# xmindflow/TransCeption

Measured on AMD Instinct MI355X. Metric: images/sec fwd+bwd at 224x224 B=16 per GPU, higher is better.
Workload: dtype bf16; 1 GPU; TransCeption (MSTransception) 224x224 B=16/GPU fwd+bwd+SGD, synthetic Synapse npz slices via the device loader, name-seeded random-init weights; global_batch=16, image_size=224, parallelism=dp1, headline_mode=loader, headline_degraded=False, launch_mode=hipGraph replay

## Files before the change

### transception_amd/_header.py

```python
from __future__ import annotations

import ctypes as C
import operator
import os
import re
from typing import NamedTuple

HEADER = os.path.join(os.path.dirname(os.path.dirname(os.path.abspath(__file__))), "include", "transception_hip.h")


class SideHeader(NamedTuple):
    attr: str
    file: str
    version: str
    entry: str
    what: str

    @property
    def path(self) -> str:
        return os.path.join(os.path.dirname(HEADER), self.file)


SIDE_HEADERS = (SideHeader("POST", "transception_post.h", "TC_POST_ABI_VERSION", "tc_post_abi_version", "post-processing"),
                SideHeader("EMA", "transception_ema.h", "TC_EMA_ABI_VERSION", "tc_ema_abi_version", "weight-averaging"),
                SideHeader("TTA", "transception_tta.h", "TC_TTA_ABI_VERSION", "tc_tta_abi_version", "test-time augmentation"),
                SideHeader("RESAMPLE", "transception_resample.h", "TC_RESAMPLE_ABI_VERSION", "tc_resample_abi_version", "score resampling"),
                SideHeader("BRIDGE", "transception_bridge.h", "TC_BRIDGE_ABI_VERSION", "tc_bridge_abi_version", "bridge LayerNorm"),
                SideHeader("LOSS", "transception_loss.h", "TC_LOSS_ABI_VERSION", "tc_loss_abi_version", "focal / Tversky loss"))

SCALARS = {"int": C.c_int, "long long": C.c_longlong, "float": C.c_float, "double": C.c_double,
           "unsigned": C.c_uint, "unsigned int": C.c_uint}
POINTEES = set(SCALARS) | {"void", "unsigned char"}


class HeaderError(ValueError):
    pass


class Function(NamedTuple):
    restype: type
    argtypes: list
    query: bool


class Header(NamedTuple):
    functions: dict
    structs: dict
    constants: dict


_TOKEN = re.compile(r"\s*(\d+|<<|[()|+-])")
_LEVELS = ({"|": operator.or_}, {"<<": operator.lshift}, {"+": operator.add, "-": operator.sub})


def evaluate(expr: str) -> int:
    toks, pos, expr = [], 0, expr.strip()
    while pos < len(expr):
        m = _TOKEN.match(expr, pos)
        if not m:
            raise HeaderError(f"constant expression {expr!r}: cannot read {expr[pos:]!r}")
# ... 122 lines not shown
```

### transception_amd/_lib.py

```python
from __future__ import annotations

import ctypes as C
import os

from . import _header

HERE = os.path.dirname(os.path.abspath(__file__))
LIB_PATH = os.environ.get("TC_LIB_PATH") or os.path.join(HERE, "libtransception_hip.so")

ABI = _header.load()
SIGNATURES = {name: f.argtypes for name, f in ABI.functions.items()}
K, S = ABI.constants, ABI.structs
SIDE = {s.attr: _header.load(s.path) for s in _header.SIDE_HEADERS}
POST, EMA, TTA, RESAMPLE, BRIDGE, LOSS = SIDE["POST"], SIDE["EMA"], SIDE["TTA"], SIDE["RESAMPLE"], SIDE["BRIDGE"], SIDE["LOSS"]

ABI_VERSION = K["TC_ABI_VERSION"]
TC_F32, TC_BF16, TC_F16 = K["TC_F32"], K["TC_BF16"], K["TC_F16"]
ACT_NONE, ACT_HSWISH, ACT_COORD, ACT_SIGMOID = K["TC_ACT_NONE"], K["TC_ACT_HSWISH"], K["TC_ACT_COORD"], K["TC_ACT_SIGMOID"]
ACT_GELU, ACT_SCALE, ACT_RELU = K["TC_ACT_GELU"], K["TC_ACT_SCALE"], K["TC_ACT_RELU"]
FFN_NONE, FFN_LN_A, FFN_LN_B, FFN_EP = K["TC_FFN_NONE"], K["TC_FFN_LN_A"], K["TC_FFN_LN_B"], K["TC_FFN_EP"]
EW_PATCHIFY, EW_DEINTERLEAVE, EW_COPY, EW_MULTI_MAX = K["TC_EW_PATCHIFY"], K["TC_EW_DEINTERLEAVE"], K["TC_EW_COPY"], K["TC_EW_MULTI_MAX"]
TC_AUG_WARP, TC_AUG_LINEAR, TC_AUG_BLUR, TC_AUG_PIECEWISE = K["TC_AUG_WARP"], K["TC_AUG_LINEAR"], K["TC_AUG_BLUR"], K["TC_AUG_PIECEWISE"]
TC_AUG_SKIP, TC_AUG_FROM_RAW = K["TC_AUG_SKIP"], K["TC_AUG_FROM_RAW"]
ATTN_DKV_SPLITS = K["TC_ATTN_DKV_SPLITS"]
TC_METRIC_NO_SOURCE, TC_METRIC_SELECT_WORK_BYTES = K["TC_METRIC_NO_SOURCE"], K["TC_METRIC_SELECT_WORK_BYTES"]
TC_IGNORE_NONE = K["TC_IGNORE_NONE"]
POST_ABI_VERSION, EMA_ABI_VERSION, TTA_ABI_VERSION, RESAMPLE_ABI_VERSION, BRIDGE_ABI_VERSION, LOSS_ABI_VERSION = (SIDE[s.attr].constants[s.version] for s in _header.SIDE_HEADERS)
TC_OVERLAP_DICE, TC_OVERLAP_TVERSKY = LOSS.constants["TC_OVERLAP_DICE"], LOSS.constants["TC_OVERLAP_TVERSKY"]
TC_CC_LARGEST, TC_CC_MIN_VOXELS = POST.constants["TC_CC_LARGEST"], POST.constants["TC_CC_MIN_VOXELS"]
TC_RESAMPLE_MAX_EXTENT = RESAMPLE.constants["TC_RESAMPLE_MAX_EXTENT"]
TC_TTA_FLIP_H, TC_TTA_FLIP_W, TC_TTA_TRANSPOSE = TTA.constants["TC_TTA_FLIP_H"], TTA.constants["TC_TTA_FLIP_W"], TTA.constants["TC_TTA_TRANSPOSE"]

TcGemm, TcLnFold, TcDwFold, TcDwSeg, TcFfnSeg = S["TcGemm"], S["TcLnFold"], S["TcDwFold"], S["TcDwSeg"], S["TcFfnSeg"]
TcFfnFused, TcFfnBwd, TcEffAtt, TcEwSeg, TcSliceAug = S["TcFfnFused"], S["TcFfnBwd"], S["TcEffAtt"], S["TcEwSeg"], S["TcSliceAug"]
TcSrSrc, TcLnSeg = BRIDGE.structs["TcSrSrc"], BRIDGE.structs["TcLnSeg"]
SR_LN_MAX, LN_MULTI_MAX = BRIDGE.constants["TC_SR_LN_MAX"], BRIDGE.constants["TC_LN_MULTI_MAX"]


class TcError(RuntimeError):
    pass


class _Lib:
    calls = 0

    def __init__(self, path: str = LIB_PATH):
        if not os.path.exists(path):
            raise TcError(f"{path} is missing: build it with `python -m transception_amd.build` "
                          "(there is no CPU/PyTorch fallback for the TransCeption hot path)")
        self.path = path
        self.cdll = C.CDLL(path)
        headers = [(ABI, "TC_ABI_VERSION", "tc_abi_version", "ABI"),
                   *((SIDE[s.attr], s.version, s.entry, s.what + " ABI") for s in _header.SIDE_HEADERS)]
        for header, *_ in headers:
            for name, f in header.functions.items():
                fn = getattr(self.cdll, name)
                fn.argtypes = f.argtypes
                fn.restype = f.restype
                setattr(self, name, fn if f.query else self._checked(name, fn))
        for header, version, entry, what in headers:
            v, host = getattr(self.cdll, entry)(), header.constants[version]
            if v != host:
                raise TcError(f"{what} mismatch: library {v}, host {host}")

    @staticmethod
    def _checked(name, fn):
        def call(*a):
            _Lib.calls += 1
            rc = fn(*a)
# ... 15 lines not shown
```

### transception_amd/build.py

```python
from __future__ import annotations

import concurrent.futures as cf
import os
import subprocess
import sys

from ._header import HEADER, SIDE_HEADERS

HERE = os.path.dirname(os.path.abspath(__file__))
CSRC = os.path.join(HERE, "csrc")
LIB = os.path.join(HERE, "libtransception_hip.so")
SOURCES = ["gemm.hip", "norm.hip", "dwconv.hip", "softmax.hip", "attention.hip", "attention_seg.hip", "elementwise.hip", "train.hip", "factoratt.hip", "data.hip", "mixffn.hip", "mixffn_bwd.hip", "effatt.hip", "cbam.hip", "ripm.hip", "linln.hip", "lncls.hip", "legacy.hip", "metrics.hip", "postprocess.hip", "ema.hip", "tta.hip", "resample.hip"]
FLAGS = ["--offload-arch=gfx950", "-O3", "-std=c++17", "-fPIC", "-ffp-contract=fast", "-munsafe-fp-atomics"]


def _hipcc() -> str:
    for c in (os.environ.get("HIPCC"), "/opt/rocm/bin/hipcc", "hipcc"):
        if c and (os.path.isabs(c) and os.path.exists(c) or not os.path.isabs(c)):
            return c
    raise RuntimeError("hipcc not found")


def _stale(target: str, deps) -> bool:
    if not os.path.exists(target):
        return True
    t = os.path.getmtime(target)
    return any(os.path.getmtime(d) > t for d in deps)


def build(force: bool = False, verbose: bool = True) -> str:
    hipcc = _hipcc()
    for gen in ("gen_attn_asm.py", "gen_dkv_asm.py", "gen_dq_asm.py"):
        r = subprocess.run([sys.executable, os.path.join(CSRC, gen)], capture_output=True, text=True)
        if r.returncode != 0:
            raise RuntimeError(f"{gen} failed:\n{r.stderr}")
    headers = [os.path.join(CSRC, "tc_common.h"), HEADER, *(s.path for s in SIDE_HEADERS)]
    extra = {"attention_seg.hip": [os.path.join(CSRC, "attn_fwd_asm.inc"), os.path.join(CSRC, "attn_dkv_asm.inc"), os.path.join(CSRC, "attn_dq_asm.inc")]}
    objdir = os.path.join(HERE, "build")
    os.makedirs(objdir, exist_ok=True)
    jobs = []
    for src in SOURCES:
        s = os.path.join(CSRC, src)
        o = os.path.join(objdir, src.replace(".hip", ".o"))
        if force or _stale(o, [s] + headers + extra.get(src, [])):
            jobs.append((s, o))
# ... 28 lines not shown
```

### transception_amd/engine.py

```python
from __future__ import annotations

import ctypes as C
import os
from typing import Callable, Dict, List, Optional, Tuple

import torch

from ._lib import (ATTN_DKV_SPLITS, EW_COPY, EW_DEINTERLEAVE, EW_PATCHIFY, TcEffAtt, TcEwSeg, TcFfnBwd, TcFfnFused, ACT_COORD, ACT_GELU, ACT_HSWISH, ACT_NONE, ACT_SCALE, ACT_SIGMOID, FFN_EP, FFN_LN_A, FFN_LN_B, TC_BF16, TC_F16, TC_F32, TcDwFold, TcDwSeg, TcFfnSeg,
                   TcGemm, TcLnFold, TcLnSeg, TcSrSrc, LN_MULTI_MAX, lib)

TC_DTYPE = {torch.float32: TC_F32, torch.bfloat16: TC_BF16, torch.float16: TC_F16}

PROFILE: Optional[dict] = None


SEG_MARKS = os.environ.get("TC_SEG_MARKS", "")
SEG_LABELS: List[str] = []


def _timed(name: str, flops: float, fn):
    if PROFILE is None:
        fn()
        return
    e0, e1 = torch.cuda.Event(enable_timing=True), torch.cuda.Event(enable_timing=True)
    e0.record()
    fn()
    e1.record()
    PROFILE.setdefault(name, []).append((e0, e1, flops))


def _gemm_work(descs):
    fl = by = 0.0
    for g in descs:
        nb = g.nb1 * g.nb2
        es = 4 if g.dtype == TC_F32 else 2
        ec = 4 if g.c_f32 else es
        fl += 2.0 * g.M * g.N * g.K * nb
        by += nb * ((g.M * g.K + g.K * g.N) * es + g.M * g.N * ec * (2 if g.accumulate else 1) + (g.M * g.N * es if g.R else 0))
    return fl, by


# ... 73 lines not shown
        return t


def _overlap(a, b) -> bool:
    return a[0] < b[1] and b[0] < a[1] and a[2] < b[3] and b[2] < a[3]


def _ptr(t: Optional[torch.Tensor]):
    return None if t is None else t.data_ptr()


_WORKSPACES: Dict[Tuple[str, str], torch.Tensor] = {}
WORKSPACE_BYTES = 16384 + 1024 * 16384


def _workspace(device, tag: str = "") -> torch.Tensor:
    key = (str(device), tag)
    ws = _WORKSPACES.get(key)
    if ws is None:
        ws = _WORKSPACES[key] = torch.zeros(WORKSPACE_BYTES * (8 if tag == "many" else 1), dtype=torch.uint8, device=device)
    return ws


_SPLITK_CAP = 128
_SPLITK_BLOCKS = 512
_SPLITK_KMIN = 384
_THR128 = 100000
_FFN_STORE_ACT = os.environ.get("TC_FFN_STORE_ACT", "1") != "0"
_FFN_LN_GEMM_MAXC = int(os.environ.get("TC_FFN_LN_GEMM_MAXC", "64"))
_FFN_TILED = os.environ.get("TC_FFN_TILED", "1") != "0"
_DW_DEFER = os.environ.get("TC_DW_DEFER", "1") != "0"
_LN_DEFER = os.environ.get("TC_LN_DEFER", "1") != "0"
_EFFATT_FUSED = os.environ.get("TC_EFFATT_FUSED", "1") != "0"
_FFN_PRE_LN = os.environ.get("TC_FFN_PRE_LN", "0") != "0"
_SR_LN_FUSED = os.environ.get("TC_SR_LN_FUSED", "1") != "0"
_LN_MULTI = os.environ.get("TC_LN_MULTI", "1") != "0"
_PENDING_RES = os.environ.get("TC_PENDING_RES", "1") != "0"
_LIN_LN_FUSED = os.environ.get("TC_LIN_LN_FUSED", "1") != "0"
_RIPM_FUSED = os.environ.get("TC_RIPM_FUSED", "1") != "0"
_LN_CLS_FUSED = os.environ.get("TC_LN_CLS_FUSED", "1") != "0"
_DW_LN_FUSED = os.environ.get("TC_DW_LN_FUSED", "1") != "0"
_MHCA_ATT_BWD_FUSED = os.environ.get("TC_MHCA_ATT_BWD_FUSED", "1") != "0"
_MHCA_ATT_FUSED = os.environ.get("TC_MHCA_ATT_FUSED", "1") != "0"
_DW_BWD_ONE = os.environ.get("TC_DW_BWD_ONE", "1") != "0"
_FFN_TILED_BWD = os.environ.get("TC_FFN_TILED_BWD", "1") != "0"
_FFN_TILE_BWD = (0, 0)
_FFN_TILE = (0, 0)
_POISON = bool(os.environ.get("TC_DEBUG_POISON"))


def _empty(shape, dtype, device) -> torch.Tensor:
    if _POISON:
        return torch.full(tuple(shape), float("nan"), dtype=dtype, device=device)
    return torch.empty(tuple(shape), dtype=dtype, device=device)


_ZERO_NEED: Dict[Tuple[str, torch.dtype], int] = {}


class _ZeroArena:
    def __init__(self, device, dtype):
        self.key = (str(device), dtype)
        self.device, self.dtype = device, dtype
        self.buf: Optional[torch.Tensor] = None
        self.used = 0
        self.asked = 0
# ... 744 lines not shown
            for nm, (W, b) in (("k", keys), ("q", queries), ("v", values), ("r", reproj)):
                setattr(f, "w" + nm, _ptr(W.data)); setattr(f, "b" + nm, _ptr(b.data))
                if grads:
                    setattr(f, "dw" + nm, _ptr(W.grad)); setattr(f, "db" + nm, _ptr(b.grad))
            if grads:
                f.dgamma, f.dbeta = _ptr(ln[0].grad), _ptr(ln[1].grad)
            f.out, f.ctx, f.kstat, f.part, f.part_floats = _ptr(out.data), _ptr(ctx), _ptr(kstat), _ptr(part), nf
            f.ldt, f.ldo, f.C, f.B, f.N, f.eps = t.ld, out.ld, Cc, B, N, eps
            if dout is not None:
                f.dout, f.lddo, f.dt, f.lddt, f.g1, f.acc_dt = _ptr(dout), dout.stride(0), _ptr(dt), dt.stride(0), _ptr(g1), acc
            return f

        part = self.f32(nf)
        f = desc(part)
        self.n_launch += 3
        _timed("hbm:effatt_fwd (LayerNorm + EfficientAttention + residual: token statistics, context fold, output)",
               3.0 * t.rows * Cc * es, lambda: L.tc_effatt_fwd(C.byref(f), self.dt, self.stream))
        del part

        def bwd():
            dy = self.grad_of(out)
            if dy is None or not t.requires_grad:
                return
            gx, acc = self.wgrad(t)
            part = self.f32(nf)
            g1 = _empty((t.rows, Cc), self.dtype, self.dev)
            fb = desc(part, dy, gx, g1, acc, grads=True)
            self.n_launch += 4
            _timed("hbm:effatt_bwd (query side + d_ctx partials, d_ctx fold, key/value side + LayerNorm backward, parameter fold)",
                   (6.0 + acc) * t.rows * Cc * es, lambda: L.tc_effatt_bwd(C.byref(fb), self.dt, self.stream))
        self._rec(bwd)
        return out

    def layernorm(self, x: Var, g: P, b: P, eps: float = 1e-5, act: int = ACT_NONE, out: Optional[Var] = None,
                  stats: Optional[Tuple[torch.Tensor, torch.Tensor]] = None, launch: bool = True) -> Var:
        Gn = self.ngroups
        rows, Cc = x.rows // Gn, x.cols
        assert Gn == 1 or (g.gs > 0 and b.gs == g.gs)
        if out is None:
            out = self.new(x.rows, Cc)
        mean, rstd = stats if stats is not None else (self.f32(x.rows), self.f32(x.rows))
        es = x.data.element_size()
        if launch:
            _timed("hbm:layernorm_fwd", 2.0 * x.rows * Cc * es, lambda: self.L.tc_layernorm_fwd(
                _ptr(x.data), x.ld, _ptr(g.data), _ptr(b.data), _ptr(out.data), out.ld, _ptr(mean), _ptr(rstd), rows, Cc, eps, act, Gn, g.gs,
                self.dt, self.stream))

        def bwd():
            dy = self.grad_of(out)
            if dy is None or not x.requires_grad:
                return
            pend = self._take_pending(x)
            gx, acc = self.wgrad(x)
            assert not (pend and acc)
            dres, ldres = (pend[0], pend[1]) if pend else (_ptr(gx) if acc else None, gx.stride(0))
            fused = g.grad is not None
            nblk = int(self.L.tc_layernorm_bwd_nblk(rows, Cc)) if (fused and _LN_DEFER) else 0
            if nblk > 0:
                nf = Gn * nblk * 2 * Cc
                part = self.f32(nf)
                _timed("hbm:layernorm_bwd", (3.0 + (dres is not None)) * x.rows * Cc * es, lambda: self.L.tc_layernorm_bwd_defer(
                    _ptr(dy), dy.stride(0), _ptr(x.data), x.ld, _ptr(g.data), _ptr(b.data), _ptr(mean), _ptr(rstd), _ptr(gx), gx.stride(0),
                    dres, ldres, _ptr(g.grad), _ptr(b.grad), rows, Cc, act, Gn, g.gs, _ptr(part), nf, self.dt,
                    self.stream))
                self._ln_pending.append((part, g.grad, b.grad, g.gs, nblk, Cc, Gn))
                if len(self._ln_pending) == 64:
# ... 1015 lines not shown
```

### transception_amd/model.py

```python
from __future__ import annotations

import math
import os
from typing import Dict, List, Optional, Tuple

import torch
import torch.nn as nn

from ._lib import ACT_COORD, ACT_GELU, ACT_HSWISH, ACT_NONE, ACT_RELU, ACT_SIGMOID, TC_F32, lib
from .engine import TC_DTYPE, Graph, P, Var

DIMS = (64, 128, 320, 512)
LAYERS = (3, 8, 3)
HEADS = 8
CRPE_WINDOW = ((3, 2), (5, 3), (7, 3))
SR_K = (8, 4, 2)
MULT = (1, 2, 5, 8)


def _xavier_convs(mod: nn.Module):
    for m in mod.modules():
        if isinstance(m, nn.Conv2d):
            nn.init.xavier_uniform_(m.weight)
            if m.bias is not None:
# ... 670 lines not shown
                residual=residual, out=out)


def _mixffn(M, G, x, name, B, H, W, residual, out=None, pre_ln=None):
    pl = (M._P(G, pre_ln[0] + ".weight"), M._P(G, pre_ln[0] + ".bias"), pre_ln[1]) if pre_ln is not None else None
    if x.data.is_contiguous():
        return G.mixffn([_mixffn_site(M, G, x, name, B, H, W, residual, out, pl)])[0]
    if pl is not None:
        x = G.layernorm(x, *pl)
    h = G.linear(x, *_lin(M, G, name + ".fc1"))
    d = G.dwconv(h, M._P(G, name + ".dwconv.dwconv.weight"), M._P(G, name + ".dwconv.dwconv.bias"), B, H, W, 3, 1, True)
    a = _ln(M, G, d, name + ".norm1", act=ACT_GELU)
    return G.linear(a, *_lin(M, G, name + ".fc2"), out=out, residual=residual)


def _mixffn_plain(M, G, x, name, B, H, W, residual, out=None):
    h = G.linear(x, *_lin(M, G, name + ".fc1"))
    d = G.dwconv(h, M._P(G, name + ".dwconv.dwconv.weight"), M._P(G, name + ".dwconv.dwconv.bias"), B, H, W, 3, 1, False)
    return G.linear(G.gelu(d), *_lin(M, G, name + ".fc2"), residual=residual, out=out)


def _eff_attention(M, G, n1: Var, name: str, B: int, N: int, residual: Optional[Var] = None, ln=None):
    C = n1.cols
    rows = B * N
    kqv = G.new(rows, 3 * C, covered=True)
    k, q, v = kqv.colslice(0, C), kqv.colslice(C, 2 * C), kqv.colslice(2 * C, 3 * C)
    lk, lq, lv = _lin(M, G, name + ".keys"), _lin(M, G, name + ".queries"), _lin(M, G, name + ".values")
    if C % 64 == 0 and G.ngroups == 1:
        G.linear_multi(n1, [lk[0], lq[0], lv[0]], [lk[1], lq[1], lv[1]], kqv)
    else:
        G.linear(n1, *lk, out=k)
        G.linear(n1, *lq, out=q)
        G.linear(n1, *lv, out=v)
    ksm = G.softmax(k, B, 0)
    qsm = G.softmax(q, 1, 1)
    ctx = G.new(B * C, C)
    G.bmm(ksm, v, ctx, C, C, N, 1, 0, nb1=B, sA=(N * ksm.ld, 0), sB=(N * v.ld, 0), sC=(C * C, 0))
    att = G.new(rows, C)
    G.bmm(qsm, ctx, att, N, C, C, 0, 0, nb1=B, sA=(N * qsm.ld, 0), sB=(C * C, 0), sC=(N * C, 0))
    return _proj_ln(M, G, att, name + ".reprojection", residual, ln)


def _eff_block(M, G, t: Var, name: str, B: int, H: int, W: int) -> Var:
    a = name + ".attn"
    blk = ((M._P(G, name + ".norm1.weight"), M._P(G, name + ".norm1.bias")), _lin(M, G, a + ".keys"), _lin(M, G, a + ".queries"),
           _lin(M, G, a + ".values"), _lin(M, G, a + ".reprojection"))
    if G.effatt_supported(t, tuple(p for pair in blk for p in pair)):
        tx = G.eff_attention_block(t, *blk, B, H * W)
        if M.token_mlp_mode == "mix":
            return _mixffn_plain(M, G, _ln(M, G, tx, name + ".norm2"), name + ".mlp", B, H, W, residual=tx)
        return _mixffn(M, G, tx, name + ".mlp", B, H, W, residual=tx, pre_ln=(name + ".norm2", 1e-5))
    tx, n2 = _eff_attention(M, G, _ln(M, G, t, name + ".norm1"), name + ".attn", B, H * W, residual=t, ln=(name + ".norm2", 1e-5))
    if M.token_mlp_mode == "mix":
        return _mixffn_plain(M, G, n2, name + ".mlp", B, H, W, residual=tx)
    return _mixffn(M, G, n2, name + ".mlp", B, H, W, residual=tx)


def _ripm(M, G, m: Var, name: str, B: int, side: int, npath: int = 3, pool: bool = True) -> Tuple[Var, int]:
    so = (side - 1) // 2 + 1 if pool else side
    rows = B * so * so
    stack = G.new(npath * rows, m.cols)
    if npath == 3 and pool and G.ripm_supported(m):
        steps = []
        for i in range(3):
            pre = f"{name}.patch_embeds.{i}.patch_conv"
            holder = M.get_submodule(pre + ".bn")
# ... 455 lines not shown
```

Measured before the change: 1520 images/sec.

## Fuse EfficientAttention core softmaxes and context products into two kernels

Adds a dedicated HIP path for the EfficientAttention core. One kernel does the token softmax of k together with the k^T v context product; a second does the channel softmax of q together with the q·ctx product. The backward pass is likewise fused into a context-gradient kernel and a per-row dq/dk/dv kernel. The goal is to remove separate softmax and batched-GEMM launches and the HBM round trips between them, in exchange for a large new hand-written MFMA kernel with shape limits (C ≤ 320, N ≤ 896). Blocks outside those limits fall back to the old path.

```diff
diff --git a/include/transception_effcore.h b/include/transception_effcore.h
--- /dev/null
+++ b/include/transception_effcore.h
@@ -0,0 +1,42 @@
+#ifndef TRANSCEPTION_EFFCORE_H
+#define TRANSCEPTION_EFFCORE_H
+
+#ifdef __cplusplus
+extern "C" {
+#endif
+
+#define TC_EFFCORE_ABI_VERSION 1
+#define TC_EFFCORE_MAX_C 320
+#define TC_EFFCORE_MAX_N 896
+#ifndef TC_QUERY
+#define TC_QUERY
+#endif
+
+TC_QUERY int tc_effcore_abi_version(void);
+
+typedef struct TcEffCore {
+    const void* k;
+    const void* q;
+    const void* v;
+    void* ksm;
+    void* qsm;
+    void* ctx;
+    void* att;
+    const void* datt;
+    void* dctx;
+    float* tpart;
+    void* dk;
+    void* dq;
+    void* dv;
+    int ldkqv, ldatt, lddatt, lddkqv;
+    int B, N, C;
+} TcEffCore;
+TC_QUERY int tc_effcore_supported(int C, int N, int dtype);
+TC_QUERY long long tc_effcore_scratch_floats(int B, int C);
+int tc_effcore_fwd(const TcEffCore* f, int dtype, void* stream);
+int tc_effcore_bwd(const TcEffCore* f, int dtype, void* stream);
+
+#ifdef __cplusplus
+}
+#endif
+#endif
diff --git a/transception_amd/_header.py b/transception_amd/_header.py
--- a/transception_amd/_header.py
+++ b/transception_amd/_header.py
@@ -26,6 +26,7 @@
                 SideHeader("TTA", "transception_tta.h", "TC_TTA_ABI_VERSION", "tc_tta_abi_version", "test-time augmentation"),
                 SideHeader("RESAMPLE", "transception_resample.h", "TC_RESAMPLE_ABI_VERSION", "tc_resample_abi_version", "score resampling"),
                 SideHeader("BRIDGE", "transception_bridge.h", "TC_BRIDGE_ABI_VERSION", "tc_bridge_abi_version", "bridge LayerNorm"),
+                SideHeader("EFFCORE", "transception_effcore.h", "TC_EFFCORE_ABI_VERSION", "tc_effcore_abi_version", "EfficientAttention core"),
                 SideHeader("LOSS", "transception_loss.h", "TC_LOSS_ABI_VERSION", "tc_loss_abi_version", "focal / Tversky loss"))
 
 SCALARS = {"int": C.c_int, "long long": C.c_longlong, "float": C.c_float, "double": C.c_double,
diff --git a/transception_amd/_lib.py b/transception_amd/_lib.py
--- a/transception_amd/_lib.py
+++ b/transception_amd/_lib.py
@@ -12,7 +12,7 @@
 SIGNATURES = {name: f.argtypes for name, f in ABI.functions.items()}
 K, S = ABI.constants, ABI.structs
 SIDE = {s.attr: _header.load(s.path) for s in _header.SIDE_HEADERS}
-POST, EMA, TTA, RESAMPLE, BRIDGE, LOSS = SIDE["POST"], SIDE["EMA"], SIDE["TTA"], SIDE["RESAMPLE"], SIDE["BRIDGE"], SIDE["LOSS"]
+POST, EMA, TTA, RESAMPLE, BRIDGE, EFFCORE, LOSS = (SIDE[s.attr] for s in _header.SIDE_HEADERS)
 
 ABI_VERSION = K["TC_ABI_VERSION"]
 TC_F32, TC_BF16, TC_F16 = K["TC_F32"], K["TC_BF16"], K["TC_F16"]
@@ -25,7 +25,7 @@
 ATTN_DKV_SPLITS = K["TC_ATTN_DKV_SPLITS"]
 TC_METRIC_NO_SOURCE, TC_METRIC_SELECT_WORK_BYTES = K["TC_METRIC_NO_SOURCE"], K["TC_METRIC_SELECT_WORK_BYTES"]
 TC_IGNORE_NONE = K["TC_IGNORE_NONE"]
-POST_ABI_VERSION, EMA_ABI_VERSION, TTA_ABI_VERSION, RESAMPLE_ABI_VERSION, BRIDGE_ABI_VERSION, LOSS_ABI_VERSION = (SIDE[s.attr].constants[s.version] for s in _header.SIDE_HEADERS)
+POST_ABI_VERSION, EMA_ABI_VERSION, TTA_ABI_VERSION, RESAMPLE_ABI_VERSION, BRIDGE_ABI_VERSION, EFFCORE_ABI_VERSION, LOSS_ABI_VERSION = (SIDE[s.attr].constants[s.version] for s in _header.SIDE_HEADERS)
 TC_OVERLAP_DICE, TC_OVERLAP_TVERSKY = LOSS.constants["TC_OVERLAP_DICE"], LOSS.constants["TC_OVERLAP_TVERSKY"]
 TC_CC_LARGEST, TC_CC_MIN_VOXELS = POST.constants["TC_CC_LARGEST"], POST.constants["TC_CC_MIN_VOXELS"]
 TC_RESAMPLE_MAX_EXTENT = RESAMPLE.constants["TC_RESAMPLE_MAX_EXTENT"]
@@ -35,6 +35,7 @@
 TcFfnFused, TcFfnBwd, TcEffAtt, TcEwSeg, TcSliceAug = S["TcFfnFused"], S["TcFfnBwd"], S["TcEffAtt"], S["TcEwSeg"], S["TcSliceAug"]
 TcSrSrc, TcLnSeg = BRIDGE.structs["TcSrSrc"], BRIDGE.structs["TcLnSeg"]
 SR_LN_MAX, LN_MULTI_MAX = BRIDGE.constants["TC_SR_LN_MAX"], BRIDGE.constants["TC_LN_MULTI_MAX"]
+TcEffCore = EFFCORE.structs["TcEffCore"]
 
 
 class TcError(RuntimeError):
diff --git a/transception_amd/build.py b/transception_amd/build.py
--- a/transception_amd/build.py
+++ b/transception_amd/build.py
@@ -10,7 +10,7 @@
 HERE = os.path.dirname(os.path.abspath(__file__))
 CSRC = os.path.join(HERE, "csrc")
 LIB = os.path.join(HERE, "libtransception_hip.so")
-SOURCES = ["gemm.hip", "norm.hip", "dwconv.hip", "softmax.hip", "attention.hip", "attention_seg.hip", "elementwise.hip", "train.hip", "factoratt.hip", "data.hip", "mixffn.hip", "mixffn_bwd.hip", "effatt.hip", "cbam.hip", "ripm.hip", "linln.hip", "lncls.hip", "legacy.hip", "metrics.hip", "postprocess.hip", "ema.hip", "tta.hip", "resample.hip"]
+SOURCES = ["gemm.hip", "norm.hip", "dwconv.hip", "softmax.hip", "attention.hip", "attention_seg.hip", "elementwise.hip", "train.hip", "factoratt.hip", "data.hip", "mixffn.hip", "mixffn_bwd.hip", "effatt.hip", "effcore.hip", "cbam.hip", "ripm.hip", "linln.hip", "lncls.hip", "legacy.hip", "metrics.hip", "postprocess.hip", "ema.hip", "tta.hip", "resample.hip"]
 FLAGS = ["--offload-arch=gfx950", "-O3", "-std=c++17", "-fPIC", "-ffp-contract=fast", "-munsafe-fp-atomics"]
 
 
diff --git a/transception_amd/csrc/effcore.hip b/transception_amd/csrc/effcore.hip
--- /dev/null
+++ b/transception_amd/csrc/effcore.hip
@@ -0,0 +1,470 @@
+#include "tc_common.h"
+#include "../../include/transception_effcore.h"
+
+namespace {
+
+constexpr int NT = 256, P64 = 72, TSL = 128, TB = 64;
+
+struct CoreDev {
+    const void* k; const void* q; const void* v;
+    void* ksm; void* qsm; void* ctx; void* att;
+    const void* datt; void* dctx; float* tpart; void* dk; void* dq; void* dv;
+    int ldkqv, ldatt, lddatt, lddkqv, B, N, C;
+};
+
+struct Lane { int lane, l31, hh, gi, gq2, wv; };
+__device__ __forceinline__ Lane lane_of() {
+    Lane L; L.lane = threadIdx.x & 63; L.wv = threadIdx.x >> 6; L.l31 = L.lane & 31; L.hh = L.lane >> 5; L.gi = L.lane & 15; L.gq2 = (L.lane >> 4) & 1;
+    return L;
+}
+__device__ __forceinline__ void zero16(tc_f32x16& a) {
+#pragma unroll
+    for (int r = 0; r < 16; ++r) a[r] = 0.f;
+}
+__device__ __forceinline__ uint4 zero4() { return make_uint4(0u, 0u, 0u, 0u); }
+
+template <typename H, int VPR, int NV> __device__ __forceinline__ void fetch_rows(uint4 (&f)[NV], const H* src, long long ld, int nvalid) {
+#pragma unroll
+    for (int i = 0; i < NV; ++i) {
+        const int idx = threadIdx.x + i * NT, r = idx / VPR, cg = idx % VPR;
+        f[i] = r < nvalid ? *reinterpret_cast<const uint4*>(src + r * ld + cg * 8) : zero4();
+    }
+}
+template <int VPR, int NV> __device__ __forceinline__ void stash_rows(bf16_t* X, int pitch, const uint4 (&f)[NV]) {
+#pragma unroll
+    for (int i = 0; i < NV; ++i) {
+        const int idx = threadIdx.x + i * NT, r = idx / VPR, cg = idx % VPR;
+        *reinterpret_cast<uint4*>(X + r * pitch + cg * 8) = f[i];
+    }
+}
+template <typename H, int VPR, int NV> __device__ __forceinline__ void store_rows(const bf16_t* X, int pitch, H* dst, long long ld, int nvalid) {
+#pragma unroll
+    for (int i = 0; i < NV; ++i) {
+        const int idx = threadIdx.x + i * NT, r = idx / VPR, cg = idx % VPR;
+        if (r < nvalid) *reinterpret_cast<uint4*>(dst + r * ld + cg * 8) = *reinterpret_cast<const uint4*>(X + r * pitch + cg * 8);
+    }
+}
+template <typename H> __device__ __forceinline__ void mm_tok(const bf16_t* X, int px, int i0, const bf16_t* Y, int py, int j0, int steps, const Lane& L, tc_f32x16& acc) {
+    using V8 = typename TcHalf<H>::v8;
+    const int col = 16 * L.gq2 + 4 * (L.gi & 3);
+    for (int ks = 0; ks < steps; ++ks) {
+        const int row = 16 * ks + 8 * L.hh + (L.gi >> 2);
+        const V8 a = tc_lds_tr8<V8>(X + row * px + i0 + col, X + (row + 4) * px + i0 + col);
+        const V8 b = tc_lds_tr8<V8>(Y + row * py + j0 + col, Y + (row + 4) * py + j0 + col);
+        acc = TcHalf<H>::mfma(a, b, acc);
+    }
+}
+template <typename H> __device__ __forceinline__ void mm_w(const bf16_t* W, int pw, int o0, const bf16_t* X, int px, int t0, int steps, const Lane& L, tc_f32x16& acc) {
+    using V8 = typename TcHalf<H>::v8;
+    const bf16_t* wr = W + (o0 + L.l31) * pw + 8 * L.hh;
+    const bf16_t* xr = X + (t0 + L.l31) * px + 8 * L.hh;
+#pragma unroll 4
+    for (int kk = 0; kk < steps; ++kk)
+        acc = TcHalf<H>::mfma(*reinterpret_cast<const V8*>(wr + kk * 16), *reinterpret_cast<const V8*>(xr + kk * 16), acc);
+}
+template <typename H, int NC> __device__ __forceinline__ void mm_wt(const bf16_t* W, int pw, int par, const bf16_t* X, int px, int t0, int x0, const Lane& L, tc_f32x16 (&acc)[NC]) {
+    using V8 = typename TcHalf<H>::v8;
+#pragma unroll
+    for (int kk = 0; kk < 4; ++kk) {
+        const V8 xv = *reinterpret_cast<const V8*>(X + (t0 + L.l31) * px + x0 + kk * 16 + 8 * L.hh);
+        const bf16_t* wp = W + (16 * kk + 8 * L.hh + (L.gi >> 2)) * pw + 16 * L.gq2 + 4 * (L.gi & 3);
+#pragma unroll
+        for (int j = 0; j < NC; ++j) {
+            const int c0 = 32 * (par + 2 * j);
+            acc[j] = TcHalf<H>::mfma(tc_lds_tr8<V8>(wp + c0, wp + 4 * pw + c0), xv, acc[j]);
+        }
+    }
+}
+template <typename H> __device__ __forceinline__ void put_T(bf16_t* X, int px, int t0, int c0, const Lane& L, const tc_f32x16& a) {
+#pragma unroll
+    for (int gq = 0; gq < 4; ++gq)
+        *reinterpret_cast<uint2*>(X + (t0 + L.l31) * px + c0 + 8 * gq + 4 * L.hh) =
+            make_uint2(pack2<H>(a[4 * gq], a[4 * gq + 1]), pack2<H>(a[4 * gq + 2], a[4 * gq + 3]));
+}
+template <typename H> __device__ __forceinline__ float4 get_T(const bf16_t* X, int px, int t0, int c0, int gq, const Lane& L) {
+    const uint2 v = *reinterpret_cast<const uint2*>(X + (t0 + L.l31) * px + c0 + 8 * gq + 4 * L.hh);
+    float4 o;
+    unpack2<H>(v.x, o.x, o.y); unpack2<H>(v.y, o.z, o.w);
+    return o;
+}
+__device__ __forceinline__ float4 f4max(float4 a, float4 b) { return make_float4(fmaxf(a.x, b.x), fmaxf(a.y, b.y), fmaxf(a.z, b.z), fmaxf(a.w, b.w)); }
+__device__ __forceinline__ float4 f4add(float4 a, float4 b) { return make_float4(a.x + b.x, a.y + b.y, a.z + b.z, a.w + b.w); }
+template <bool MAX> __device__ __forceinline__ float4 block_reduce16(float4 v, float4 (*sm)[16], int tx, int ty) {
+    sm[ty][tx] = v;
+    __syncthreads();
+    float4 r = sm[0][tx];
+#pragma unroll
+    for (int i = 1; i < 16; ++i) r = MAX ? f4max(r, sm[i][tx]) : f4add(r, sm[i][tx]);
+    __syncthreads();
+    return r;
+}
+template <typename H> __device__ __forceinline__ float4 lds4(const bf16_t* p) {
+    const uint2 v = *reinterpret_cast<const uint2*>(p);
+    float4 o;
+    unpack2<H>(v.x, o.x, o.y); unpack2<H>(v.y, o.z, o.w);
+    return o;
+}
+template <typename H> __device__ __forceinline__ uint2 pk4(float4 v) { return make_uint2(pack2<H>(v.x, v.y), pack2<H>(v.z, v.w)); }
+
+template <typename H, int NTOK>
+__global__ __launch_bounds__(NT) void effcore_ctx_kernel(const CoreDev p) {
+    __shared__ __attribute__((aligned(16))) bf16_t kt[NTOK * P64], vt[TSL * P64];
+    __shared__ float4 red[16][16];
+    const int kb = blockIdx.x, vb = blockIdx.y, b = blockIdx.z, N = p.N, tid = threadIdx.x;
+    const long long ld = p.ldkqv;
+    const H* K = reinterpret_cast<const H*>(p.k) + (long long)b * N * ld + kb * 64;
+    const H* V = reinterpret_cast<const H*>(p.v) + (long long)b * N * ld + vb * 64;
+    const int ns = (N + TSL - 1) / TSL, nvec = ns * TSL * 8;
+    uint4 vf[4], vg[4];
+    fetch_rows<H, 8, 4>(vf, V, ld, N);
+    if (ns > 1) fetch_rows<H, 8, 4>(vg, V + (long long)TSL * ld, ld, N - TSL);
+    for (int base = 0; base < nvec; base += NT * 8) {
+        uint4 t[8];
+#pragma unroll
+        for (int j = 0; j < 8; ++j) {
+            const int idx = base + j * NT + tid, r = idx >> 3;
+            t[j] = (idx < nvec && r < N) ? *reinterpret_cast<const uint4*>(K + r * ld + (idx & 7) * 8) : zero4();
+        }
+#pragma unroll
+        for (int j = 0; j < 8; ++j) {
+            const int idx = base + j * NT + tid;
+            if (idx < nvec) *reinterpret_cast<uint4*>(kt + (idx >> 3) * P64 + (idx & 7) * 8) = t[j];
+        }
+    }
+    __syncthreads();
+    const int tx = tid & 15, ty = tid >> 4;
+    float4 m = make_float4(-INFINITY, -INFINITY, -INFINITY, -INFINITY);
+    for (int r0 = ty; r0 < N; r0 += 128) {
+        float4 x[8];
+#pragma unroll
+        for (int j = 0; j < 8; ++j) x[j] = lds4<H>(kt + min(r0 + 16 * j, N - 1) * P64 + tx * 4);
+#pragma unroll
+        for (int j = 0; j < 8; ++j) m = f4max(m, x[j]);
+    }
+    m = block_reduce16<true>(m, red, tx, ty);
+    float4 s = make_float4(0.f, 0.f, 0.f, 0.f);
+    for (int r0 = ty; r0 < N; r0 += 128) {
+        float4 x[8];
+#pragma unroll
+        for (int j = 0; j < 8; ++j) x[j] = lds4<H>(kt + min(r0 + 16 * j, N - 1) * P64 + tx * 4);
+#pragma unroll
+        for (int j = 0; j < 8; ++j)
+            if (r0 + 16 * j < N) { s.x += __expf(x[j].x - m.x); s.y += __expf(x[j].y - m.y); s.z += __expf(x[j].z - m.z); s.w += __expf(x[j].w - m.w); }
+    }
+    s = block_reduce16<false>(s, red, tx, ty);
+    s.x = 1.f / s.x; s.y = 1.f / s.y; s.z = 1.f / s.z; s.w = 1.f / s.w;
+    H* KS = reinterpret_cast<H*>(p.ksm) + (long long)b * N * p.C + kb * 64 + tx * 4;
+    for (int r0 = ty; r0 < N; r0 += 128) {
+        float4 x[8];
+#pragma unroll
+        for (int j = 0; j < 8; ++j) x[j] = lds4<H>(kt + min(r0 + 16 * j, N - 1) * P64 + tx * 4);
+#pragma unroll
+        for (int j = 0; j < 8; ++j) {
+            const int r = r0 + 16 * j;
+            if (r < N) {
+                float4 y = x[j];
+                y.x = __expf(y.x - m.x) * s.x; y.y = __expf(y.y - m.y) * s.y; y.z = __expf(y.z - m.z) * s.z; y.w = __expf(y.w - m.w) * s.w;
+                const uint2 o = pk4<H>(y);
+                *reinterpret_cast<uint2*>(kt + r * P64 + tx * 4) = o;
+                if (vb == 0) *reinterpret_cast<uint2*>(KS + (long long)r * p.C) = o;
+            }
+        }
+    }
+    const Lane L = lane_of();
+    const int ib = L.wv >> 1, jb = L.wv & 1;
+    tc_f32x16 acc;
+    zero16(acc);
+    for (int sl = 0; sl < ns; sl += 2) {
+        stash_rows<8, 4>(vt, P64, vf);
+        if (sl + 2 < ns) fetch_rows<H, 8, 4>(vf, V + (long long)(sl + 2) * TSL * ld, ld, N - (sl + 2) * TSL);
+        TC_LDS_BARRIER();
+        mm_tok<H>(kt + sl * TSL * P64, P64, ib * 32, vt, P64, jb * 32, TSL / 16, L, acc);
+        TC_LDS_BARRIER();
+        if (sl + 1 < ns) {
+            stash_rows<8, 4>(vt, P64, vg);
+            if (sl + 3 < ns) fetch_rows<H, 8, 4>(vg, V + (long long)(sl + 3) * TSL * ld, ld, N - (sl + 3) * TSL);
+            TC_LDS_BARRIER();
+            mm_tok<H>(kt + (sl + 1) * TSL * P64, P64, ib * 32, vt, P64, jb * 32, TSL / 16, L, acc);
+            TC_LDS_BARRIER();
+        }
+    }
+    H* CX = reinterpret_cast<H*>(p.ctx) + ((long long)b * p.C + kb * 64 + ib * 32) * p.C + vb * 64 + jb * 32 + L.l31;
+#pragma unroll
+    for (int r = 0; r < 16; ++r) stf<H>(CX + ((r & 3) + 8 * (r >> 2) + 4 * L.hh) * p.C, acc[r]);
+}
+
+template <typename H, int NC>
+__global__ __launch_bounds__(NT) void effcore_att_kernel(const CoreDev p) {
+    constexpr int C = 64 * NC, PC = C + 8, VPR = 8 * NC;
+    __shared__ __attribute__((aligned(16))) bf16_t qt[TB * PC], cs[64 * PC];
+    const int blk = blockIdx.x, b = blockIdx.y, N = p.N, tid = threadIdx.x;
+    const int nv = min(TB, N - blk * TB);
+    const long long row0 = (long long)b * N + blk * TB;
+    const H* CX = reinterpret_cast<const H*>(p.ctx) + (long long)b * C * C;
+    uint4 cf[2 * NC];
+    fetch_rows<H, VPR, 2 * NC>(cf, CX, C, 64);
+    {
+        const int row = tid >> 2, sub = tid & 3;
+        const bool ok = row < nv;
+        const H* Q = reinterpret_cast<const H*>(p.q) + (row0 + row) * p.ldkqv;
+        uint4 raw[2 * NC];
+#pragma unroll
+        for (int i = 0; i < 2 * NC; ++i) raw[i] = ok ? *reinterpret_cast<const uint4*>(Q + (sub + 4 * i) * 8) : zero4();
+        float x[2 * NC][8];
+        float m = -INFINITY;
+#pragma unroll
+        for (int i = 0; i < 2 * NC; ++i) {
+            tc_unpack16<H>(raw[i], x[i]);
+#pragma unroll
+            for (int e = 0; e < 8; ++e) m = fmaxf(m, x[i][e]);
+        }
+        m = tc_group_max<4>(m);
+        float s = 0.f;
+#pragma unroll
+        for (int i = 0; i < 2 * NC; ++i)
+#pragma unroll
+            for (int e = 0; e < 8; ++e) { x[i][e] = __expf(x[i][e] - m); s += x[i][e]; }
+        s = 1.0f / tc_group_sum<4>(s);
+        H* QS = reinterpret_cast<H*>(p.qsm) + (row0 + row) * C;
+#pragma unroll
+        for (int i = 0; i < 2 * NC; ++i) {
+#pragma unroll
+            for (int e = 0; e < 8; ++e) x[i][e] *= s;
+            const uint4 o = ok ? tc_pack16<H>(x[i]) : zero4();
+            if (ok) *reinterpret_cast<uint4*>(QS + (sub + 4 * i) * 8) = o;
+            *reinterpret_cast<uint4*>(qt + row * PC + (sub + 4 * i) * 8) = o;
+        }
+    }
+    const Lane L = lane_of();
+    const int th = L.wv & 1, par = L.wv >> 1;
+    tc_f32x16 acc[NC];
+#pragma unroll
+    for (int j = 0; j < NC; ++j) zero16(acc[j]);
+    for (int sl = 0; sl < NC; ++sl) {
+        stash_rows<VPR, 2 * NC>(cs, PC, cf);
+        if (sl + 1 < NC) fetch_rows<H, VPR, 2 * NC>(cf, CX + (long long)(sl + 1) * 64 * C, C, 64);
+        TC_LDS_BARRIER();
+        mm_wt<H, NC>(cs, PC, par, qt, PC, th * 32, sl * 64, L, acc);
+        TC_LDS_BARRIER();
+    }
+#pragma unroll
+    for (int j = 0; j < NC; ++j) put_T<H>(qt, PC, th * 32, 32 * (par + 2 * j), L, acc[j]);
+    TC_LDS_BARRIER();
+    store_rows<H, VPR, 2 * NC>(qt, PC, reinterpret_cast<H*>(p.att) + row0 * p.ldatt, p.ldatt, nv);
+}
+
+template <typename H>
+__global__ __launch_bounds__(NT) void effcore_dctx_kernel(const CoreDev p) {
+    __shared__ __attribute__((aligned(16))) bf16_t xt[TSL * P64], yt[TSL * P64];
+    __shared__ float ts[2][2][32];
+    const int cb = blockIdx.x, vb = blockIdx.y, b = blockIdx.z, N = p.N, C = p.C;
+    const H* X = reinterpret_cast<const H*>(p.qsm) + (long long)b * N * C + cb * 64;
+    const H* Y = reinterpret_cast<const H*>(p.datt) + (long long)b * N * p.lddatt + vb * 64;
+    const int ns = (N + TSL - 1) / TSL;
+    const Lane L = lane_of();
+    const int ib = L.wv >> 1, jb = L.wv & 1;
+    uint4 xf[4], yf[4];
+    fetch_rows<H, 8, 4>(xf, X, C, N);
+    fetch_rows<H, 8, 4>(yf, Y, p.lddatt, N);
+    const long long tile = ((long long)b * C + cb * 64 + ib * 32) * C + vb * 64 + jb * 32 + L.l31;
+    const H* CX = reinterpret_cast<const H*>(p.ctx) + tile;
+    float cx[16];
+#pragma unroll
+    for (int r = 0; r < 16; ++r) cx[r] = ldf<H>(CX + ((r & 3) + 8 * (r >> 2) + 4 * L.hh) * C);
+    tc_f32x16 acc;
+    zero16(acc);
+    for (int sl = 0; sl < ns; ++sl) {
+        stash_rows<8, 4>(xt, P64, xf);
+        stash_rows<8, 4>(yt, P64, yf);
+        if (sl + 1 < ns) {
+            fetch_rows<H, 8, 4>(xf, X + (long long)(sl + 1) * TSL * C, C, N - (sl + 1) * TSL);
+            fetch_rows<H, 8, 4>(yf, Y + (long long)(sl + 1) * TSL * p.lddatt, p.lddatt, N - (sl + 1) * TSL);
+        }
+        TC_LDS_BARRIER();
+        mm_tok<H>(xt, P64, ib * 32, yt, P64, jb * 32, TSL / 16, L, acc);
+        TC_LDS_BARRIER();
+    }
+    H* DC = reinterpret_cast<H*>(p.dctx) + tile;
+#pragma unroll
+    for (int r = 0; r < 16; ++r) {
+        const int i = (r & 3) + 8 * (r >> 2) + 4 * L.hh;
+        H o;
+        stf<H>(&o, acc[r]);
+        DC[i * C] = o;
+        const float pr = tc_group_sum<32>(cx[r] * ldf<H>(&o));
+        if (L.l31 == 0) ts[ib][jb][i] = pr;
+    }
+    __syncthreads();
+    if (threadIdx.x < 64) {
+        const int i2 = threadIdx.x >> 5, i = threadIdx.x & 31;
+        p.tpart[((long long)b * (C / 64) + vb) * C + cb * 64 + threadIdx.x] = ts[i2][0][i] + ts[i2][1][i];
+    }
+}
+
+template <typename H, int NC>
+__global__ __launch_bounds__(NT) void effcore_rows_kernel(const CoreDev p) {
+    constexpr int C = 64 * NC, PC = C + 8, VPR = 8 * NC;
+    __shared__ __attribute__((aligned(16))) bf16_t tile[TB * PC], slab[64 * PC], ks[TB * P64], dks[TB * P64];
+    __shared__ float dots[2][TB];
+    __shared__ __attribute__((aligned(16))) float tv[64];
+    const int blk = blockIdx.x, b = blockIdx.y, N = p.N, tid = threadIdx.x;
+    const int nv = min(TB, N - blk * TB);
+    const long long row0 = (long long)b * N + blk * TB;
+    const Lane L = lane_of();
+    const int th = L.wv & 1, ch = L.wv >> 1;
+    uint4 cf[2 * NC], tf[2 * NC];
+    if (blockIdx.z == 0) {
+    const H* CX = reinterpret_cast<const H*>(p.ctx) + (long long)b * C * C;
+    fetch_rows<H, VPR, 2 * NC>(tf, reinterpret_cast<const H*>(p.datt) + row0 * p.lddatt, p.lddatt, nv);
+    fetch_rows<H, VPR, 2 * NC>(cf, CX, C, 64);
+    stash_rows<VPR, 2 * NC>(tile, PC, tf);
+    fetch_rows<H, VPR, 2 * NC>(tf, reinterpret_cast<const H*>(p.qsm) + row0 * C, C, nv);
+    tc_f32x16 kept[NC];
+#pragma unroll
+    for (int sl = 0; sl < NC; ++sl) {
+        stash_rows<VPR, 2 * NC>(slab, PC, cf);
+        if (sl + 1 < NC) fetch_rows<H, VPR, 2 * NC>(cf, CX + (long long)(sl + 1) * 64 * C, C, 64);
+        TC_LDS_BARRIER();
+        zero16(kept[sl]);
+        mm_w<H>(slab, PC, ch * 32, tile, PC, th * 32, C / 16, L, kept[sl]);
+        TC_LDS_BARRIER();
+    }
+    stash_rows<VPR, 2 * NC>(slab, PC, tf);
+    TC_LDS_BARRIER();
+    float dot = 0.f;
+#pragma unroll
+    for (int sl = 0; sl < NC; ++sl)
+#pragma unroll
+        for (int gq = 0; gq < 4; ++gq) {
+            const float4 qv = get_T<H>(slab, PC, th * 32, sl * 64 + ch * 32, gq, L);
+            dot += qv.x * kept[sl][4 * gq] + qv.y * kept[sl][4 * gq + 1] + qv.z * kept[sl][4 * gq + 2] + qv.w * kept[sl][4 * gq + 3];
+        }
+    dot += __shfl_xor(dot, 32, 64);
+    if (L.hh == 0) dots[ch][th * 32 + L.l31] = dot;
+    TC_LDS_BARRIER();
+    dot = dots[0][th * 32 + L.l31] + dots[1][th * 32 + L.l31];
+#pragma unroll
+    for (int sl = 0; sl < NC; ++sl) {
+#pragma unroll
+        for (int gq = 0; gq < 4; ++gq) {
+            const float4 qv = get_T<H>(slab, PC, th * 32, sl * 64 + ch * 32, gq, L);
+            kept[sl][4 * gq] = qv.x * (kept[sl][4 * gq] - dot); kept[sl][4 * gq + 1] = qv.y * (kept[sl][4 * gq + 1] - dot);
+            kept[sl][4 * gq + 2] = qv.z * (kept[sl][4 * gq + 2] - dot); kept[sl][4 * gq + 3] = qv.w * (kept[sl][4 * gq + 3] - dot);
+        }
+        put_T<H>(tile, PC, th * 32, sl * 64 + ch * 32, L, kept[sl]);
+    }
+    TC_LDS_BARRIER();
+    store_rows<H, VPR, 2 * NC>(tile, PC, reinterpret_cast<H*>(p.dq) + row0 * p.lddkqv, p.lddkqv, nv);
+    return;
+    }
+    const H* DCX = reinterpret_cast<const H*>(p.dctx) + (long long)b * C * C;
+    fetch_rows<H, VPR, 2 * NC>(tf, reinterpret_cast<const H*>(p.v) + row0 * p.ldkqv, p.ldkqv, nv);
+    fetch_rows<H, VPR, 2 * NC>(cf, DCX, C, 64);
+    stash_rows<VPR, 2 * NC>(tile, PC, tf);
+    const H* KSM = reinterpret_cast<const H*>(p.ksm) + row0 * C;
+    uint4 kf[2];
+    fetch_rows<H, 8, 2>(kf, KSM, C, nv);
+    const float* TP = p.tpart + (long long)b * NC * C;
+    tc_f32x16 dv[NC];
+#pragma unroll
+    for (int j = 0; j < NC; ++j) zero16(dv[j]);
+#pragma unroll 1
+    for (int sl = 0; sl < NC; ++sl) {
+        stash_rows<VPR, 2 * NC>(slab, PC, cf);
+        stash_rows<8, 2>(ks, P64, kf);
+        if (tid < 64) {
+            float t = 0.f;
+#pragma unroll
+            for (int j = 0; j < NC; ++j) t += TP[j * C + sl * 64 + tid];
+            tv[tid] = t;
+        }
+        if (sl + 1 < NC) {
+            fetch_rows<H, VPR, 2 * NC>(cf, DCX + (long long)(sl + 1) * 64 * C, C, 64);
+            fetch_rows<H, 8, 2>(kf, KSM + (sl + 1) * 64, C, nv);
+        }
+        TC_LDS_BARRIER();
+        tc_f32x16 a;
+        zero16(a);
+        mm_w<H>(slab, PC, ch * 32, tile, PC, th * 32, C / 16, L, a);
+#pragma unroll
+        for (int gq = 0; gq < 4; ++gq) {
+            const float4 kv = get_T<H>(ks, P64, th * 32, ch * 32, gq, L);
+            const float4 t4 = *reinterpret_cast<const float4*>(tv + ch * 32 + 8 * gq + 4 * L.hh);
+            a[4 * gq] = kv.x * (a[4 * gq] - t4.x); a[4 * gq + 1] = kv.y * (a[4 * gq + 1] - t4.y);
+            a[4 * gq + 2] = kv.z * (a[4 * gq + 2] - t4.z); a[4 * gq + 3] = kv.w * (a[4 * gq + 3] - t4.w);
+        }
+        put_T<H>(dks, P64, th * 32, ch * 32, L, a);
+        mm_wt<H, NC>(slab, PC, ch, ks, P64, th * 32, 0, L, dv);
+        TC_LDS_BARRIER();
+        store_rows<H, 8, 2>(dks, P64, reinterpret_cast<H*>(p.dk) + row0 * p.lddkqv + sl * 64, p.lddkqv, nv);
+    }
+#pragma unroll
+    for (int j = 0; j < NC; ++j) put_T<H>(tile, PC, th * 32, 32 * (ch + 2 * j), L, dv[j]);
+    TC_LDS_BARRIER();
+    store_rows<H, VPR, 2 * NC>(tile, PC, reinterpret_cast<H*>(p.dv) + row0 * p.lddkqv, p.lddkqv, nv);
+}
+
+bool al16(const void* q) { return q && !((uintptr_t)q & 15); }
+bool core_ok(const TcEffCore* f, int dtype, bool bwd) {
+    if (!f || !tc_effcore_supported(f->C, f->N, dtype) || f->B < 1 || f->B > 65535) return false;
+    if (!al16(f->k) || !al16(f->q) || !al16(f->v) || !al16(f->ksm) || !al16(f->qsm) || !al16(f->ctx) || !al16(f->att)) return false;
+    if ((f->ldkqv & 7) || (f->ldatt & 7) || f->ldkqv < f->C || f->ldatt < f->C) return false;
+    if ((long long)f->B * f->N * (f->ldkqv > f->ldatt ? f->ldkqv : f->ldatt) >= 0x7fffffffLL) return false;
+    if (!bwd) return true;
+    if (!al16(f->datt) || !al16(f->dctx) || !al16(f->tpart) || !al16(f->dk) || !al16(f->dq) || !al16(f->dv)) return false;
+    if ((f->lddatt & 7) || (f->lddkqv & 7) || f->lddatt < f->C || f->lddkqv < f->C) return false;
+    return (long long)f->B * f->N * (f->lddkqv > f->lddatt ? f->lddkqv : f->lddatt) < 0x7fffffffLL;
+}
+CoreDev core_dev(const TcEffCore* f) {
+    CoreDev p;
+    p.k = f->k; p.q = f->q; p.v = f->v; p.ksm = f->ksm; p.qsm = f->qsm; p.ctx = f->ctx; p.att = f->att;
+    p.datt = f->datt; p.dctx = f->dctx; p.tpart = f->tpart; p.dk = f->dk; p.dq = f->dq; p.dv = f->dv;
+    p.ldkqv = f->ldkqv; p.ldatt = f->ldatt; p.lddatt = f->lddatt; p.lddkqv = f->lddkqv; p.B = f->B; p.N = f->N; p.C = f->C;
+    return p;
+}
+
+#define TC_CORE_NC(K, ...)                                                  \
+    switch (NCv) {                                                         \
+        case 1: hipLaunchKernelGGL((K<H, 1>), __VA_ARGS__); break;         \
+        case 2: hipLaunchKernelGGL((K<H, 2>), __VA_ARGS__); break;         \
+        case 3: hipLaunchKernelGGL((K<H, 3>), __VA_ARGS__); break;         \
+        case 4: hipLaunchKernelGGL((K<H, 4>), __VA_ARGS__); break;         \
+        default: hipLaunchKernelGGL((K<H, 5>), __VA_ARGS__); break;        \
+    }
+
+template <typename H> int core_fwd(const TcEffCore* f, hipStream_t s) {
+    const CoreDev p = core_dev(f);
+    const int NCv = f->C / 64, nblk = (f->N + TB - 1) / TB;
+    const dim3 g1(NCv, NCv, f->B);
+    if (f->N <= 256) hipLaunchKernelGGL((effcore_ctx_kernel<H, 256>), g1, dim3(NT), 0, s, p);
+    else hipLaunchKernelGGL((effcore_ctx_kernel<H, TC_EFFCORE_MAX_N>), g1, dim3(NT), 0, s, p);
+    if (tc_launch_status() != TC_OK) return TC_ERR_LAUNCH;
+    TC_CORE_NC(effcore_att_kernel, dim3(nblk, f->B), dim3(NT), 0, s, p)
+    return tc_launch_status();
+}
+template <typename H> int core_bwd(const TcEffCore* f, hipStream_t s) {
+    const CoreDev p = core_dev(f);
+    const int NCv = f->C / 64, nblk = (f->N + TB - 1) / TB;
+    hipLaunchKernelGGL((effcore_dctx_kernel<H>), dim3(NCv, NCv, f->B), dim3(NT), 0, s, p);
+    if (tc_launch_status() != TC_OK) return TC_ERR_LAUNCH;
+    TC_CORE_NC(effcore_rows_kernel, dim3(nblk, f->B, 2), dim3(NT), 0, s, p)
+    return tc_launch_status();
+}
+
+static_assert(TC_EFFCORE_MAX_N % TSL == 0 && TC_EFFCORE_MAX_C == 320, "the k tile holds whole slabs; the NC switch ends at 5");
+
+}
+
+extern "C" int tc_effcore_abi_version(void) { return TC_EFFCORE_ABI_VERSION; }
+extern "C" int tc_effcore_supported(int C, int N, int dtype) {
+    return (dtype == TC_BF16 || dtype == TC_F16) && C >= 64 && C <= TC_EFFCORE_MAX_C && C % 64 == 0 && N >= 1 && N <= TC_EFFCORE_MAX_N;
+}
+extern "C" long long tc_effcore_scratch_floats(int B, int C) { return (B > 0 && C > 0 && C % 64 == 0) ? (long long)B * (C / 64) * C : 0; }
+extern "C" int tc_effcore_fwd(const TcEffCore* f, int dtype, void* stream) {
+    if (!core_ok(f, dtype, false)) return TC_ERR_ARG;
+    return dtype == TC_BF16 ? core_fwd<bf16_t>(f, (hipStream_t)stream) : core_fwd<f16_t>(f, (hipStream_t)stream);
+}
+extern "C" int tc_effcore_bwd(const TcEffCore* f, int dtype, void* stream) {
+    if (!core_ok(f, dtype, true)) return TC_ERR_ARG;
+    return dtype == TC_BF16 ? core_bwd<bf16_t>(f, (hipStream_t)stream) : core_bwd<f16_t>(f, (hipStream_t)stream);
+}
diff --git a/transception_amd/engine.py b/transception_amd/engine.py
--- a/transception_amd/engine.py
+++ b/transception_amd/engine.py
@@ -6,7 +6,7 @@
 
 import torch
 
-from ._lib import (ATTN_DKV_SPLITS, EW_COPY, EW_DEINTERLEAVE, EW_PATCHIFY, TcEffAtt, TcEwSeg, TcFfnBwd, TcFfnFused, ACT_COORD, ACT_GELU, ACT_HSWISH, ACT_NONE, ACT_SCALE, ACT_SIGMOID, FFN_EP, FFN_LN_A, FFN_LN_B, TC_BF16, TC_F16, TC_F32, TcDwFold, TcDwSeg, TcFfnSeg,
+from ._lib import (ATTN_DKV_SPLITS, EW_COPY, EW_DEINTERLEAVE, EW_PATCHIFY, TcEffAtt, TcEffCore, TcEwSeg, TcFfnBwd, TcFfnFused, ACT_COORD, ACT_GELU, ACT_HSWISH, ACT_NONE, ACT_SCALE, ACT_SIGMOID, FFN_EP, FFN_LN_A, FFN_LN_B, TC_BF16, TC_F16, TC_F32, TcDwFold, TcDwSeg, TcFfnSeg,
                    TcGemm, TcLnFold, TcLnSeg, TcSrSrc, LN_MULTI_MAX, lib)
 
 TC_DTYPE = {torch.float32: TC_F32, torch.bfloat16: TC_BF16, torch.float16: TC_F16}
@@ -146,6 +146,7 @@
 _DW_DEFER = os.environ.get("TC_DW_DEFER", "1") != "0"
 _LN_DEFER = os.environ.get("TC_LN_DEFER", "1") != "0"
 _EFFATT_FUSED = os.environ.get("TC_EFFATT_FUSED", "1") != "0"
+_EFFCORE_FUSED = os.environ.get("TC_EFFCORE_FUSED", "1") != "0"
 _FFN_PRE_LN = os.environ.get("TC_FFN_PRE_LN", "0") != "0"
 _SR_LN_FUSED = os.environ.get("TC_SR_LN_FUSED", "1") != "0"
 _LN_MULTI = os.environ.get("TC_LN_MULTI", "1") != "0"
@@ -956,6 +957,51 @@
         self._rec(bwd)
         return out
 
+    def effcore_supported(self, k: Var, q: Var, v: Var, B: int, N: int) -> bool:
+        if self.record and not (k.requires_grad and q.requires_grad and v.requires_grad):
+            return False
+        Cc = k.cols
+        return (_EFFCORE_FUSED and self.ngroups == 1 and self.dt != TC_F32 and q.cols == Cc and v.cols == Cc
+                and k.rows == q.rows == v.rows == B * N and k.ld == q.ld == v.ld and k.ld % 8 == 0
+                and all(x.data.data_ptr() % 16 == 0 for x in (k, q, v)) and bool(self.L.tc_effcore_supported(Cc, N, self.dt)))
+
+    def eff_attention_core(self, k: Var, q: Var, v: Var, B: int, N: int) -> Var:
+        L, Cc, rows = self.L, k.cols, B * N
+        assert self.effcore_supported(k, q, v, B, N)
+        att = self.new(rows, Cc)
+        ksm, qsm = _empty((rows, Cc), self.dtype, self.dev), _empty((rows, Cc), self.dtype, self.dev)
+        ctx = _empty((B * Cc, Cc), self.dtype, self.dev)
+        es = k.data.element_size()
+
+        def desc():
+            f = TcEffCore()
+            f.k, f.q, f.v, f.ldkqv = _ptr(k.data), _ptr(q.data), _ptr(v.data), k.ld
+            f.ksm, f.qsm, f.ctx, f.att, f.ldatt = _ptr(ksm), _ptr(qsm), _ptr(ctx), _ptr(att.data), att.ld
+            f.B, f.N, f.C = B, N, Cc
+            return f
+
+        f = desc()
+        self.n_launch += 2
+        _timed("hbm:effcore_fwd (token softmax of k + context product, channel softmax of q + attended map)",
+               6.0 * rows * Cc * es, lambda: L.tc_effcore_fwd(C.byref(f), self.dt, self.stream))
+
+        def bwd():
+            datt = self.grad_of(att)
+            if datt is None:
+                return
+            (gk, ak), (gq, aq), (gv, av) = self.wgrad(k), self.wgrad(q), self.wgrad(v)
+            assert not (ak or aq or av) and gk.stride(0) == gq.stride(0) == gv.stride(0), "the core's backward writes dk, dq, dv once"
+            fb = desc()
+            dctx = _empty((B * Cc, Cc), self.dtype, self.dev)
+            tpart = self.f32(int(L.tc_effcore_scratch_floats(B, Cc)))
+            fb.datt, fb.lddatt, fb.dctx, fb.tpart = _ptr(datt), datt.stride(0), _ptr(dctx), _ptr(tpart)
+            fb.dk, fb.dq, fb.dv, fb.lddkqv = _ptr(gk), _ptr(gq), _ptr(gv), gk.stride(0)
+            self.n_launch += 2
+            _timed("hbm:effcore_bwd (context gradient + column-softmax sums, dq | dk | dv by token rows)",
+                   9.0 * rows * Cc * es, lambda: L.tc_effcore_bwd(C.byref(fb), self.dt, self.stream))
+        self._rec(bwd)
+        return att
+
     def layernorm(self, x: Var, g: P, b: P, eps: float = 1e-5, act: int = ACT_NONE, out: Optional[Var] = None,
                   stats: Optional[Tuple[torch.Tensor, torch.Tensor]] = None, launch: bool = True) -> Var:
         Gn = self.ngroups
diff --git a/transception_amd/model.py b/transception_amd/model.py
--- a/transception_amd/model.py
+++ b/transception_amd/model.py
@@ -726,6 +726,8 @@
         G.linear(n1, *lk, out=k)
         G.linear(n1, *lq, out=q)
         G.linear(n1, *lv, out=v)
+    if G.effcore_supported(k, q, v, B, N):
+        return _proj_ln(M, G, G.eff_attention_core(k, q, v, B, N), name + ".reprojection", residual, ln)
     ksm = G.softmax(k, B, 0)
     qsm = G.softmax(q, 1, 1)
     ctx = G.new(B * C, C)
```

Measured after the change: 1487 images/sec. 0.979x the previous value.
